# mathcom/G2Vec

Measured on NVIDIA H100. Metric: cbow_context_windows_per_sec, higher is better.
Workload: dtype f32

## Files before the change

### g2vec_b200/_capi.py

```python
import ctypes
import os

from . import build as _build

_lib = None

_vp, _i32, _i64, _u32, _u64, _f32 = (ctypes.c_void_p, ctypes.c_int32, ctypes.c_int64, ctypes.c_uint32,
                                     ctypes.c_uint64, ctypes.c_float)

SIGNATURES = {
    "g2v_abi_version": (ctypes.c_int, []),
    "g2v_last_error": (ctypes.c_char_p, []),
    "g2v_device_info": (ctypes.c_int, [_vp, _vp, _vp, _vp]),
    "g2v_launch_count": (_i64, []),
    "g2v_walk_workspace_bytes": (ctypes.c_size_t, []),
    "g2v_walk_launch": (ctypes.c_int, [_vp, _vp, _vp, _i32, _i64, _i32, _u64, _u32, _i64, _i64, _i64,
                                       _vp, _vp, _vp, _vp]),
    "g2v_walk_packed_bytes": (ctypes.c_int, [_i32, _i64, _vp, _vp]),
    "g2v_walk_prepare": (ctypes.c_int, [_vp, _vp, _vp, _i32, _i64, _vp, _vp, _vp, _vp, _vp]),
    "g2v_walk_launch_packed": (ctypes.c_int, [_vp, _vp, _i32, _i32, _i64, _i32, _u64, _u32, _i64, _i64, _i64,
                                              _vp, _vp, _vp, _vp, _vp]),
    "g2v_walk_host": (ctypes.c_int, [_vp, _vp, _vp, _i32, _i64, _i32, _u64, _u32, _i64, _i64, _i64, _vp, _vp]),
    "g2v_cbow_fwdbwd": (ctypes.c_int, [_vp, _vp, _vp, _vp, _i64, _i64, _f32, _vp, _vp, _vp, _vp, _vp, _vp,
                                       _i32, _i32, _i32, _vp]),
# ... 13 lines not shown
    "g2v_cbow_batch_expand": (ctypes.c_int, [_vp, _vp, _vp, _vp, _i64, _vp, _vp, _i32, _i32, _i32, _vp]),
    "g2v_cbow_epoch_order": (ctypes.c_int, [_vp, _i64, _u64, _i32, _i64, _i64, _vp, _vp]),
    "g2v_cbow_batch_plan_workspace_bytes": (ctypes.c_size_t, [_i64, _i64, _i64, _i32]),
    "g2v_cbow_batch_plan": (ctypes.c_int, [_vp, _vp, _vp, _i64, _i64, _i64, _i32, _vp, _vp, _vp, _vp, _vp, _vp]),
    "g2v_cbow_update": (ctypes.c_int, [_vp, _vp, _vp, _vp, _vp, _vp, _vp, _vp, _i32, _i32, _i32, _f32, _f32,
                                       _f32, _f32, _i32, _vp, _vp]),
    "g2v_cbow_update_nvl": (ctypes.c_int, [_vp, _vp, _vp, _vp, _vp, _vp, _i64, _i32, _i32, _i32, _f32, _f32, _f32,
                                           _f32, _i32, _vp, _vp]),
    "g2v_cbow_adam_tick": (ctypes.c_int, [_vp, _f32, _f32, _f32, _vp]),
    "g2v_cbow_eval": (ctypes.c_int, [_vp, _vp, _vp, _vp, _i64, _i64, _vp, _vp, _vp, _i32, _i32, _i32, _vp]),
    "g2v_cbow_loop_init": (ctypes.c_int, [_vp, _i64, _i32, _vp]),
    "g2v_cbow_loop_attach": (ctypes.c_int, [_vp]),
    "g2v_cbow_loop_begin": (ctypes.c_int, [_vp, _vp, _vp, _vp, _i64, _vp]),
    "g2v_cbow_loop_tail": (ctypes.c_int, [_vp, _vp, _vp, _vp, _vp, _i64, _f32, _vp, _vp, _vp, _vp, _vp, _i32, _i32, _i32,
                                          _vp]),
    "g2v_cbow_loop_decide": (ctypes.c_int, [_vp, _vp, _vp, _vp]),
    "g2v_cbow_loop_counters_nvl": (ctypes.c_int, [_vp, _vp, _vp, _vp, _i32, _vp]),
    "g2v_cbow_slab_plan": (ctypes.c_int, [_i32, _i32, _vp]),
    "g2v_cbow_slab_workspace_bytes": (ctypes.c_size_t, [_i64, _i32, _i32]),
    "g2v_cbow_slab_setup": (ctypes.c_int, [_vp, _vp, _vp, _i64, _i64, _i32, _i32, _vp, _vp]),
    "g2v_cbow_fwdbwd_slabs": (ctypes.c_int, [_vp, _vp, _vp, _i64, _i64, _f32, _vp, _vp, _vp, _vp, _vp, _vp,
                                             _i32, _i32, _i32, _i32, _vp, _vp]),
    "g2v_cbow_eval_slabs": (ctypes.c_int, [_vp, _vp, _vp, _i64, _i64, _vp, _vp, _vp, _i32, _i32, _i32, _i32, _vp, _vp]),
    "g2v_cbow_step_host": (ctypes.c_int, [_vp, _vp, _vp, _i64, _i64, _vp, _vp, _vp, _vp, _vp, _vp, _i32, _i32,
                                          _i32, _i32, _f32, _f32, _f32, _f32, _i32, _vp, _vp]),
    "g2v_cbow_r1_prepare": (ctypes.c_int, [_vp, _vp, _vp, _i32, _i32, _vp]),
    "g2v_cbow_r1_windows": (ctypes.c_int, [_vp, _vp, _vp, _vp, _i64, _i64, _f32, _vp, _vp, _vp, _vp, _i32, _i32, _vp]),
    "g2v_cbow_r1_windows_csc": (ctypes.c_int, [_vp, _vp, _vp, _vp, _i64, _f32, _vp, _vp, _vp, _vp, _vp, _vp, _vp,
                                              _i32, _i32, _vp]),
    "g2v_cbow_r1_scratch_bytes": (ctypes.c_size_t, [_i32]),
    "g2v_cbow_r1_update": (ctypes.c_int, [_vp, _vp, _vp, _vp, _vp, _vp, _vp, _vp, _vp, _i32, _i32, _i32, _f32, _f32,
                                         _f32, _f32, _i32, _vp, _vp]),
    "g2v_pcc_zscore": (ctypes.c_int, [_vp, _i32, _i32, _vp, _vp]),
    "g2v_pcc_edge_weights": (ctypes.c_int, [_vp, _i32, _i32, _vp, _vp, _i64, _vp, _vp]),
    "g2v_paths_canonicalise": (ctypes.c_int, [_vp, _i64, _i32, _vp, _vp, _vp]),
    "g2v_paths_mark": (ctypes.c_int, [_vp, _vp, _vp, _vp, _i64, _i32, _vp, _vp]),
    "g2v_paths_set_workspace_bytes": (ctypes.c_size_t, [_i64]),
    "g2v_paths_set_select": (ctypes.c_int, [_vp, _vp, _vp, _vp, _i64, _i32, _vp, _vp, _vp, _vp]),
    "g2v_paths_set_emit": (ctypes.c_int, [_vp, _vp, _vp, _vp, _i64, _i32, _i32, _vp, _i64, _i64, _vp, _vp, _vp, _vp,
                                          _vp, _vp]),
    "g2v_test_l2_rows": (ctypes.c_int, [_vp, _vp, _vp, _i64, _i32, _i32, _vp, _vp]),
    "g2v_test_draws": (ctypes.c_int, [_u64, _u64, _i32, _vp, _vp]),
    "g2v_test_curand_draws": (ctypes.c_int, [_u64, _u64, _i32, _vp, _vp]),
}

OPT_ADAM_TF1, OPT_SGD = 0, 1
REDUCE_SUM, REDUCE_MEAN = 0, 1
# ... 39 lines not shown
```

### g2vec_b200/cbow.py

```python
import math
import time

import numpy as np
import torch

from . import _capi


def split_indices(n, seed):
    perm = np.arange(n, dtype=np.int64)
    np.random.RandomState(seed).shuffle(perm)
    pivot = int(n * 0.8)
    return perm[:pivot], perm[pivot:]


def truncated_normal(shape, stddev, rng):
    x = rng.standard_normal(size=shape)
    bad = np.abs(x) > 2.0
    while bad.any():
        x[bad] = rng.standard_normal(size=int(bad.sum()))
        bad = np.abs(x) > 2.0
    return (x * stddev).astype(np.float32)


# ... 114 lines not shown
        if n == 0:
            return
        ptr = win.data_ptr()
        for k in [k for k in self._batches if k[0] == ptr]:
            del self._batches[k]
        key = (ptr, n, B)
        for k in [k for k in self._plan_bufs if k[0] == ptr and k != key]:
            del self._plan_bufs[k]
        buf = self._plan_bufs.get(key)
        if buf is None:
            buf = _PlanBuffers(self, win, B)
            self._plan_bufs[key] = buf
        rows, segptr, pos, brp = buf.build(win)
        data = (win, rows, segptr, pos)
        for k in range(brp.shape[0] - 1):
            self._batches[(ptr, k * B, min(B, n - k * B))] = (data, int(brp[k]), int(brp[k + 1] - brp[k]))
        if self._dO is None or self._dO.shape[0] < B:
            self._dO = torch.empty(B, dtype=torch.float32, device=self.device)
        self._pending = None

    def batch_touched(self, win, win_begin, n):
        return self._batches[(self._ptr(win), int(win_begin), int(n))][2]

    def prepare_slabs(self, win, win_begin=0, n_win=None):
        if self.algo != "rows" or self.det:
            return False
        import ctypes
        if not hasattr(self, "_n_slabs"):
            s = ctypes.c_int32(1)
            _capi.check(self.lib.g2v_cbow_slab_plan(self.V, self.D, ctypes.byref(s)), "g2v_cbow_slab_plan")
            self._n_slabs, self._slabs = int(s.value), {}
        n = ((win.shape[0] if win is not None else self.rowptr.shape[0] - 1) - win_begin) if n_win is None else n_win
        if self._n_slabs <= 1 or n <= 0:
            return False
        ws = torch.empty(int(self.lib.g2v_cbow_slab_workspace_bytes(int(n), self.D, self._n_slabs)), dtype=torch.uint8,
                         device=self.device)
        _capi.check(self.lib.g2v_cbow_slab_setup(self.rowptr.data_ptr(), self.gene.data_ptr(), self._ptr(win),
                                                 int(win_begin), int(n), self.V, self._n_slabs, ws.data_ptr(),
                                                 self._stream()), "g2v_cbow_slab_setup")
        self._slabs[(self._ptr(win), int(win_begin), int(n))] = ws
        return True

    def _slab_ws(self, win, win_begin, n):
        slabs = getattr(self, "_slabs", None)
        return slabs.get((self._ptr(win), int(win_begin), int(n))) if slabs else None

    def grad_tensors(self):
        if self.nvl:
            return []
        return [self.g_flat] if self.algo == "rows" else [self.c]

    def exchange(self):
        if self.nvl:
            return "nvl-multicast (multimem.ld_reduce / multimem.st)" if self.nvl["g_mc"] else "nvl-p2p (peer loads / stores)"
        return "nccl all_reduce"

    def _stream(self):
        return torch.cuda.current_stream(self.device).cuda_stream

    @staticmethod
    def _ptr(t):
        return 0 if t is None else t.data_ptr()

    def _csc_for(self, win, win_begin, n):
        csc = getattr(self, "_csc", None)
        if csc is not None and win is not None and csc[0] == win.data_ptr() and win_begin == 0 and n == csc[1]:
            return csc
        return None
# ... 12 lines not shown
                rc = self.lib.g2v_cbow_r1_windows_csc(self.rowptr.data_ptr(), self.gene.data_ptr(),
                                                      self.label.data_ptr(), win.data_ptr(), int(n),
                                                      1.0 / float(n_total), self.s.data_ptr(), csc[2].data_ptr(),
                                                      csc[3].data_ptr(), csc[4].data_ptr(), self.c.data_ptr(),
                                                      self.acc.data_ptr(), self.acc.data_ptr() + 8, self.V,
                                                      self.reduce, self._stream())
                _capi.check(rc, "g2v_cbow_r1_windows_csc")
                return
            rc = self.lib.g2v_cbow_r1_windows(self.rowptr.data_ptr(), self.gene.data_ptr(), self.label.data_ptr(),
                                              self._ptr(win), int(win_begin), int(n), 1.0 / float(n_total),
                                              self.s.data_ptr(), self.c.data_ptr(), self.acc.data_ptr(),
                                              self.acc.data_ptr() + 8, self.V, self.reduce, self._stream())
            _capi.check(rc, "g2v_cbow_r1_windows")
            return
        ws = self._slab_ws(win, win_begin, n)
        if ws is not None:
            rc = self.lib.g2v_cbow_fwdbwd_slabs(self.gene.data_ptr(), self.label.data_ptr(), self._ptr(win),
                                                int(win_begin), int(n), 1.0 / float(n_total), self.W_ih.data_ptr(),
                                                self.W_ho.data_ptr(), self.g_ih.data_ptr(), self.g_ho.data_ptr(),
                                                self.acc.data_ptr(), self.acc.data_ptr() + 8, self.V, self.D,
                                                self.reduce, self._n_slabs, ws.data_ptr(), self._stream())
            _capi.check(rc, "g2v_cbow_fwdbwd_slabs")
            return
        if csc is not None:
            rc = self.lib.g2v_cbow_fwdbwd_csc(self.rowptr.data_ptr(), self.gene.data_ptr(), self.label.data_ptr(),
                                              win.data_ptr(), int(n), 1.0 / float(n_total), self.W_ih.data_ptr(),
                                              self.W_ho.data_ptr(), csc[2].data_ptr(), csc[3].data_ptr(),
                                              csc[4].data_ptr(), self.g_ih.data_ptr(), self.g_ho.data_ptr(),
                                              self.acc.data_ptr(), self.acc.data_ptr() + 8, self.V, self.D,
                                              self.reduce, self._stream())
            _capi.check(rc, "g2v_cbow_fwdbwd_csc")
            return
        rc = self.lib.g2v_cbow_fwdbwd(self.rowptr.data_ptr(), self.gene.data_ptr(), self.label.data_ptr(),
                                      self._ptr(win), int(win_begin), int(n), 1.0 / float(n_total),
                                      self.W_ih.data_ptr(), self.W_ho.data_ptr(), self.g_ih.data_ptr(),
                                      self.g_ho.data_ptr(), self.acc.data_ptr(), self.acc.data_ptr() + 8,
                                      self.V, self.D, self.reduce, self._stream())
        _capi.check(rc, "g2v_cbow_fwdbwd")

    def _plan(self, win, win_begin, n):
        plan = self._batches.get((self._ptr(win), int(win_begin), int(n)))
        if plan is None:
            raise RuntimeError("%s: windows [%d, %d) of this list were not given to prepare_batches"
                               % ("optimizer='lazy_adam'" if self.lazy else "deterministic=True", win_begin, win_begin + n))
        return plan

# ... 86 lines not shown
            nv["hg"].barrier(channel=1)
            return
        rc = self.lib.g2v_cbow_update(self.W_ih.data_ptr(), self.W_ho.data_ptr(), self._ptr(self.m_ih),
                                      self._ptr(self.v_ih), self._ptr(self.m_ho), self._ptr(self.v_ho),
                                      self.g_ih.data_ptr(), self.g_ho.data_ptr(), self.V, self.D, self.opt,
                                      self.lr, self.beta1, self.beta2, self.eps, self.t, adev, self._stream())
        _capi.check(rc, "g2v_cbow_update")

    def evaluate(self, win, slot, win_begin=0, n_win=None):
        n = (win.shape[0] - win_begin) if n_win is None else n_win
        if self.algo == "rank1":
            rc = self.lib.g2v_cbow_r1_windows(self.rowptr.data_ptr(), self.gene.data_ptr(), self.label.data_ptr(),
                                              self._ptr(win), int(win_begin), int(n), 0.0, self.s.data_ptr(), 0, 0,
                                              self.acc.data_ptr() + 8 * slot, self.V, self.reduce, self._stream())
            _capi.check(rc, "g2v_cbow_r1_windows")
            return
        ws = self._slab_ws(win, win_begin, n)
        if ws is not None:
            rc = self.lib.g2v_cbow_eval_slabs(self.gene.data_ptr(), self.label.data_ptr(), self._ptr(win),
                                              int(win_begin), int(n), self.W_ih.data_ptr(), self.W_ho.data_ptr(),
                                              self.acc.data_ptr() + 8 * slot, self.V, self.D, self.reduce,
                                              self._n_slabs, ws.data_ptr(), self._stream())
            _capi.check(rc, "g2v_cbow_eval_slabs")
            return
        rc = self.lib.g2v_cbow_eval(self.rowptr.data_ptr(), self.gene.data_ptr(), self.label.data_ptr(),
                                    self._ptr(win), int(win_begin), int(n), self.W_ih.data_ptr(),
                                    self.W_ho.data_ptr(), self.acc.data_ptr() + 8 * slot, self.V, self.D,
                                    self.reduce, self._stream())
        _capi.check(rc, "g2v_cbow_eval")

    def loss_sum(self, acc_host):
        return float(acc_host[:1].view(torch.float64)[0])


def _nvl_setup(group, n_flat, dev):
    import os
    import sys
    if os.environ.get("G2V_CBOW_NVL", "1") == "0":
        return None
    try:
        import torch.distributed as dist
        import torch.distributed._symmetric_memory as symm
        w = symm.empty(n_flat, dtype=torch.float32, device=dev)
        g = symm.empty(n_flat, dtype=torch.float32, device=dev)
        hw, hg = symm.rendezvous(w, group), symm.rendezvous(g, group)
        mc = os.environ.get("G2V_CBOW_NVL_MULTICAST", "1") != "0"
# ... 263 lines not shown
                                            None if self.result is None else self.result.data_ptr(), m.V * m.D,
                                            self._st()), "g2v_cbow_loop_begin")
        if self.n_tr_loc:
            m.fwdbwd(self.tr_d, self.n_tr)
        if m_fb is not None:
            m_fb.record()
        if dist:
            for g in m.grad_tensors():
                dist.all_reduce(g)
        m.update()
        if m_upd is not None:
            m_upd.record()
        if self.n_va_loc:
            m.evaluate(self.va_d, 2)
        if m_val is not None:
            m_val.record()
        if self.carried and m.det:
            _capi.check(lib.g2v_cbow_loop_tail_det(self.ctl.data_ptr(), m.rowptr.data_ptr(), m.gene.data_ptr(),
                                                   m.label.data_ptr(), self.tr_d.data_ptr(), self.n_tr_loc,
                                                   1.0 / float(self.n_tr), m.W_ih.data_ptr(), m.W_ho.data_ptr(),
                                                   m._csc[4].data_ptr(), m.g_ho.data_ptr(), m.acc.data_ptr(), m.V, m.D,
                                                   m.reduce, m.det_workspace(self.n_tr_loc).data_ptr(), 0, self._st()),
                        "g2v_cbow_loop_tail_det")
        elif self.carried:
            csc = m._csc
            _capi.check(lib.g2v_cbow_loop_tail(self.ctl.data_ptr(), m.rowptr.data_ptr(), m.gene.data_ptr(),
                                               m.label.data_ptr(), self.tr_d.data_ptr(), self.n_tr_loc,
                                               1.0 / float(self.n_tr), m.W_ih.data_ptr(), m.W_ho.data_ptr(),
                                               csc[4].data_ptr(), m.g_ho.data_ptr(), m.acc.data_ptr(), m.V, m.D,
                                               m.reduce, self._st()), "g2v_cbow_loop_tail")
        elif show and self.n_tr_loc:
            m.evaluate(self.tr_d, 3)
        acc_ptr = m.acc.data_ptr()
        if self.hist_nvl:
            hn = self.hist_nvl
            _capi.check(lib.g2v_cbow_loop_counters_nvl(self.ctl.data_ptr(), acc_ptr, hn["h"].buffer_ptrs_dev, hn["mc"],
                                                       m.nvl["world"], self._st()), "g2v_cbow_loop_counters_nvl")
            hn["h"].barrier(channel=3)
            acc_ptr = None
        elif dist:
            dist.all_reduce(m.acc[1:4])
        _capi.check(lib.g2v_cbow_loop_decide(self.ctl.data_ptr(), acc_ptr, self.hist_d.data_ptr(), self._st()),
                    "g2v_cbow_loop_decide")

    def fetch(self):
        self.ctl_pin.copy_(self.ctl, non_blocking=True)
# ... 142 lines not shown
```

### g2vec_b200/csrc/g2v_cbow.cu

```cuda
#include "g2v_cbow_common.cuh"

namespace g2v {

constexpr int kRowsEval = 0, kRowsScatter = 1, kRowsCsc = 2;

template <int VEC, int MODE>
__global__ void __launch_bounds__(kCbowWarps * 32)
cbow_rows_kernel(const int32_t *__restrict__ rowptr, const int32_t *__restrict__ gene,
                 const uint8_t *__restrict__ label, const int32_t *__restrict__ win,
                 int64_t win_begin, int64_t n_win, float inv_n, const float *__restrict__ W_ih,
                 const float *__restrict__ W_ho, float *__restrict__ g_ih, float *__restrict__ g_ho,
                 double *__restrict__ loss_sum, unsigned long long *__restrict__ n_correct,
                 int32_t reduce_mean, const int32_t *__restrict__ skip, float *__restrict__ dO_pos,
                 const int32_t *__restrict__ carried) {
    G2V_SKIP_IF_STOPPED(skip);
    G2V_SKIP_IF_STOPPED(carried);
    constexpr bool BACKWARD = MODE != kRowsEval;
    constexpr int D = 128 * VEC;
    constexpr int D4 = D / 4;
    constexpr int UNR = 8 / VEC;
    __shared__ float sh_gho[BACKWARD ? D : 1];
    __shared__ CtaAcc sh_acc;
    const int lane = threadIdx.x & 31, warp = threadIdx.x >> 5;
    if (BACKWARD) for (int i = threadIdx.x; i < D; i += blockDim.x) sh_gho[i] = 0.f;
// ... 814 lines not shown
}

extern "C" int g2v_cbow_fwd_do(const int32_t *rowptr, const int32_t *gene, const uint8_t *label, const int32_t *win,
                               int64_t n_win, float inv_n_total, const float *W_ih, const float *W_ho, float *dO,
                               float *g_ho, double *loss_sum, int64_t *n_correct, int32_t V, int32_t D, int32_t reduce,
                               void *stream) {
    G2V_REQUIRE(V > 0 && D > 0 && n_win >= 0, "g2v_cbow_fwd_do: bad sizes (V=%d D=%d n_win=%lld)", V, D, (long long)n_win);
    G2V_REQUIRE(rowptr && label && W_ih && W_ho && dO && g_ho, "g2v_cbow_fwd_do: null pointer");
    G2V_REQUIRE(reduce == G2V_REDUCE_SUM || reduce == G2V_REDUCE_MEAN, "g2v_cbow_fwd_do: unknown reduce %d", reduce);
    if (n_win == 0) return 0;
    return launch_rows<true>(rowptr, gene, label, win, 0, n_win, inv_n_total, W_ih, W_ho, nullptr, g_ho, loss_sum,
                             n_correct, D, reduce, (cudaStream_t)stream, dO);
}

extern "C" int g2v_cbow_loop_tail(int64_t *ctl, const int32_t *rowptr, const int32_t *gene, const uint8_t *label,
                                  const int32_t *win, int64_t n_win, float inv_n_total, const float *W_ih,
                                  const float *W_ho, float *dO, float *g_ho, int64_t *acc, int32_t V, int32_t D,
                                  int32_t reduce, void *stream) {
    G2V_REQUIRE(ctl && acc, "g2v_cbow_loop_tail: null loop state");
    cudaStream_t st = (cudaStream_t)stream;
    int rc = g2v_cbow_fwd_do(rowptr, gene, label, win, n_win, inv_n_total, W_ih, W_ho, dO, g_ho,
                             reinterpret_cast<double *>(acc + 4), acc + 5, V, D, reduce, st);
    if (rc) return rc;
    loop_carry_kernel<<<1, 1, 0, st>>>(reinterpret_cast<long long *>(ctl), reinterpret_cast<long long *>(acc));
    G2V_CUDA_OK(cudaGetLastError());
    count_launch();
    return 0;
}

extern "C" size_t g2v_cbow_det_workspace_bytes(int64_t n_win, int32_t D) {
    if (n_win < 0 || D <= 0) return 0;
    const int64_t n_tiles = (n_win + kDetTile - 1) / kDetTile;
    return det_ws_loss_bytes(n_tiles) + (size_t)n_tiles * (size_t)D * sizeof(float);
}

#define G2V_DET_CHECK(name)                                                                                            \
    G2V_REQUIRE(V > 0 && D > 0 && n_win >= 0 && max_ctas >= 0, name ": bad sizes (V=%d D=%d n_win=%lld max_ctas=%d)", \
                V, D, (long long)n_win, max_ctas);                                                                     \
    G2V_REQUIRE(n_win == 0 || (rowptr && gene && label && win && W_ih && W_ho && dO && g_ho && workspace),            \
                name ": null pointer");                                                                                \
    G2V_REQUIRE(reduce == G2V_REDUCE_SUM || reduce == G2V_REDUCE_MEAN, name ": unknown reduce %d", reduce)

extern "C" int g2v_cbow_fwdbwd_csc_det(const int32_t *rowptr, const int32_t *gene, const uint8_t *label,
                                       const int32_t *win, int64_t n_win, float inv_n_total, const float *W_ih,
                                       const float *W_ho, const int32_t *cscptr, const int32_t *csc_pos, float *dO,
                                       float *g_ih, float *g_ho, double *loss_sum, int64_t *n_correct, int32_t V,
// ... 14 lines not shown
}

extern "C" int g2v_cbow_fwd_do_det(const int32_t *rowptr, const int32_t *gene, const uint8_t *label,
                                   const int32_t *win, int64_t n_win, float inv_n_total, const float *W_ih,
                                   const float *W_ho, float *dO, float *g_ho, double *loss_sum, int64_t *n_correct,
                                   int32_t V, int32_t D, int32_t reduce, void *workspace, int32_t max_ctas,
                                   void *stream) {
    G2V_DET_CHECK("g2v_cbow_fwd_do_det");
    if (n_win == 0) return 0;
    return launch_rows_det(rowptr, gene, label, win, n_win, inv_n_total, W_ih, W_ho, dO, g_ho, loss_sum, n_correct, D,
                           reduce, workspace, max_ctas, (cudaStream_t)stream, nullptr);
}
#undef G2V_DET_CHECK

extern "C" int g2v_cbow_loop_tail_det(int64_t *ctl, const int32_t *rowptr, const int32_t *gene, const uint8_t *label,
                                      const int32_t *win, int64_t n_win, float inv_n_total, const float *W_ih,
                                      const float *W_ho, float *dO, float *g_ho, int64_t *acc, int32_t V, int32_t D,
                                      int32_t reduce, void *workspace, int32_t max_ctas, void *stream) {
    G2V_REQUIRE(ctl && acc, "g2v_cbow_loop_tail_det: null loop state");
    cudaStream_t st = (cudaStream_t)stream;
    int rc = g2v_cbow_fwd_do_det(rowptr, gene, label, win, n_win, inv_n_total, W_ih, W_ho, dO, g_ho,
                                 reinterpret_cast<double *>(acc + 4), acc + 5, V, D, reduce, workspace, max_ctas, st);
    if (rc) return rc;
    loop_carry_kernel<<<1, 1, 0, st>>>(reinterpret_cast<long long *>(ctl), reinterpret_cast<long long *>(acc));
    G2V_CUDA_OK(cudaGetLastError());
    count_launch();
    return 0;
}

extern "C" int g2v_cbow_batch_expand(const int32_t *rows, const int32_t *segptr, const int32_t *pos, const float *dO,
                                     int64_t n_rows, const float *W_ho, float *g_ih, int32_t V, int32_t D,
                                     int32_t max_ctas, void *stream) {
    G2V_REQUIRE(V > 0 && D > 0 && n_rows >= 0 && n_rows <= V && max_ctas >= 0,
                "g2v_cbow_batch_expand: bad sizes (V=%d D=%d n_rows=%lld max_ctas=%d)", V, D, (long long)n_rows, max_ctas);
    G2V_REQUIRE(n_rows == 0 || (rows && segptr && pos && dO && W_ho && g_ih), "g2v_cbow_batch_expand: null pointer");
    if (n_rows == 0) return 0;
    int grid = 0, rc;
    if ((rc = det_grid((const void *)cbow_batch_expand_kernel, 0, n_rows, max_ctas, &grid))) return rc;
    cbow_batch_expand_kernel<<<grid, kCbowWarps * 32, 0, (cudaStream_t)stream>>>(rows, segptr, pos, dO, n_rows, W_ho,
                                                                                  g_ih, D, loop_skip_flag());
    G2V_CUDA_OK(cudaGetLastError());
    count_launch();
    return 0;
}

extern "C" int g2v_cbow_eval(const int32_t *rowptr, const int32_t *gene, const uint8_t *label,
                             const int32_t *win, int64_t win_begin, int64_t n_win, const float *W_ih,
                             const float *W_ho, int64_t *n_correct, int32_t V, int32_t D, int32_t reduce,
                             void *stream) {
    G2V_REQUIRE(V > 0 && D > 0 && n_win >= 0 && win_begin >= 0, "g2v_cbow_eval: bad sizes");
// ... 169 lines not shown
```

### g2vec_b200/csrc/g2v_cbow_common.cuh

```cuda
#pragma once
#include "g2v_common.cuh"

namespace g2v {

constexpr int kCbowWarps = 8;

__device__ __forceinline__ float4 ldg4(const float4 *p) { return __ldg(p); }
__device__ __forceinline__ void red_add4(float *p, float4 v) {
    asm volatile("red.global.add.v4.f32 [%0], {%1, %2, %3, %4};" ::"l"(p), "f"(v.x), "f"(v.y), "f"(v.z),
                 "f"(v.w)
                 : "memory");
}
__device__ __forceinline__ float sigmoid_stable(float x) {
    if (x >= 0.f) { const float z = expf(-x); return 1.f / (1.f + z); }
    const float z = expf(x);
    return z / (1.f + z);
}

__device__ __forceinline__ void adam1(float &w, float &m, float &v, float g, float alpha, float omb1,
                                      float omb2, float eps) {
    m += (g - m) * omb1;
    v += (g * g - v) * omb2;
    w -= (m * alpha) / (sqrtf(v) + eps);
}
// ... 16 lines not shown
    constexpr int D = 128 * VEC;
    if (TRAIN && ACTIVE) {
#pragma unroll
        for (int v = 0; v < VEC; ++v) {
            float *p = sh_gho + (v * 32 + lane) * 4;
            atomicAdd(p + 0, gho[v].x); atomicAdd(p + 1, gho[v].y);
            atomicAdd(p + 2, gho[v].z); atomicAdd(p + 3, gho[v].w);
        }
    }
    if (ACTIVE && lane == 0) {
        if (TRAIN) atomicAdd(&sh_acc.loss, (double)loss_acc);
        atomicAdd(&sh_acc.correct, (unsigned long long)correct_acc);
    }
    __syncthreads();
    if (TRAIN && ACTIVE) for (int i = threadIdx.x; i < D; i += blockDim.x) atomicAdd(g_ho + i, sh_gho[i]);
    if (ACTIVE && threadIdx.x == 0) {
        if (TRAIN && loss_sum) atomicAdd(loss_sum, sh_acc.loss);
        if (n_correct) atomicAdd(n_correct, sh_acc.correct);
    }
}

int rows_grid(const void *kernel, size_t smem, int64_t n_items, int *grid_out);

}
```

### include/g2vec_b200.h

```cpp
#ifndef G2VEC_B200_H
#define G2VEC_B200_H

#include <stddef.h>
#include <stdint.h>

#ifdef __cplusplus
extern "C" {
#endif

#define G2V_ABI_VERSION 2

#define G2V_OPT_ADAM_TF1 0
#define G2V_OPT_SGD 1

#define G2V_REDUCE_SUM 0
#define G2V_REDUCE_MEAN 1

int g2v_abi_version(void);
const char *g2v_last_error(void);

int g2v_device_info(int32_t *sm_count, int32_t *cc_major, int32_t *cc_minor, int64_t *l2_bytes);
int64_t g2v_launch_count(void);

size_t g2v_walk_workspace_bytes(void);
// ... 78 lines not shown

int g2v_cbow_loop_init(int64_t *ctl, int64_t max_steps, int32_t early_stop, void *stream);
int g2v_cbow_loop_attach(const int64_t *ctl);
int g2v_cbow_loop_begin(const int64_t *ctl, int64_t *acc, const float *W_ih, float *snapshot, int64_t n, void *stream);
int g2v_cbow_loop_tail(int64_t *ctl, const int32_t *rowptr, const int32_t *gene, const uint8_t *label,
                       const int32_t *win, int64_t n_win, float inv_n_total, const float *W_ih, const float *W_ho,
                       float *dO, float *g_ho, int64_t *acc, int32_t V, int32_t D, int32_t reduce, void *stream);
int g2v_cbow_loop_decide(int64_t *ctl, const int64_t *acc, int64_t *hist, void *stream);
int g2v_cbow_loop_counters_nvl(const int64_t *ctl, const int64_t *acc, int64_t *const *hist_ptrs_dev,
                               int64_t *hist_multicast, int32_t world, void *stream);

int g2v_cbow_slab_plan(int32_t V, int32_t D, int32_t *n_slabs);
size_t g2v_cbow_slab_workspace_bytes(int64_t n_win, int32_t D, int32_t n_slabs);
int g2v_cbow_slab_setup(const int32_t *rowptr, const int32_t *gene, const int32_t *win, int64_t win_begin,
                        int64_t n_win, int32_t V, int32_t n_slabs, void *workspace, void *stream);
int g2v_cbow_fwdbwd_slabs(const int32_t *gene, const uint8_t *label, const int32_t *win, int64_t win_begin,
                          int64_t n_win, float inv_n_total, const float *W_ih, const float *W_ho, float *g_ih,
                          float *g_ho, double *loss_sum, int64_t *n_correct, int32_t V, int32_t D, int32_t reduce,
                          int32_t n_slabs, void *workspace, void *stream);
int g2v_cbow_eval_slabs(const int32_t *gene, const uint8_t *label, const int32_t *win, int64_t win_begin,
                        int64_t n_win, const float *W_ih, const float *W_ho, int64_t *n_correct, int32_t V,
                        int32_t D, int32_t reduce, int32_t n_slabs, void *workspace, void *stream);

int g2v_cbow_step_host(const int32_t *rowptr, const int32_t *gene, const uint8_t *label,
                       int64_t n_win, int64_t nnz, float *W_ih, float *W_ho, float *m_ih,
                       float *v_ih, float *m_ho, float *v_ho, int32_t V, int32_t D,
                       int32_t optimizer, int32_t reduce, float lr, float beta1, float beta2,
                       float eps, int32_t t, double *loss_sum, int64_t *n_correct);

int g2v_cbow_r1_prepare(const float *W_ih, const float *W_ho, float *s, int32_t V, int32_t D,
                        void *stream);
int g2v_cbow_r1_windows(const int32_t *rowptr, const int32_t *gene, const uint8_t *label,
                        const int32_t *win, int64_t win_begin, int64_t n_win, float inv_n_total,
                        const float *s, float *c, double *loss_sum, int64_t *n_correct, int32_t V,
                        int32_t reduce, void *stream);
int g2v_cbow_r1_windows_csc(const int32_t *rowptr, const int32_t *gene, const uint8_t *label,
                            const int32_t *win, int64_t n_win, float inv_n_total, const float *s,
                            const int32_t *cscptr, const int32_t *csc_pos, float *dO, float *c,
                            double *loss_sum, int64_t *n_correct, int32_t V, int32_t reduce, void *stream);
size_t g2v_cbow_r1_scratch_bytes(int32_t D);
int g2v_cbow_r1_update(float *W_ih, float *W_ho, float *m_ih, float *v_ih, float *m_ho, float *v_ho,
                       float *c, float *g_ho, float *s, int32_t V, int32_t D, int32_t optimizer,
                       float lr, float beta1, float beta2, float eps, int32_t t, const float *alpha_dev,
                       void *stream);

int g2v_pcc_zscore(const float *expr, int32_t S, int32_t V, float *z, void *stream);
// ... 26 lines not shown
```

Measured before the change: 153.3 million.

## Add vocabulary-partitioned CBOW forward that stages W_ih row blocks in shared memory

Adds a partitioned CBOW path for vocabularies that fit in a single slab. The path splits the vocabulary into row ranges that fit in shared memory and precomputes per-window split points. Each CTA loads one partition of W_ih into shared memory and sums the partial hidden-output dot products for every window, pulling work chunks through atomic tickets and then moving on to the least-loaded partition. A finish kernel combines the per-partition partial outputs. This replaces scattered global gathers of embedding rows with shared-memory reads, at the cost of a setup pass, extra workspace, and a host sync during setup.

```diff
diff --git a/g2vec_b200/_capi.py b/g2vec_b200/_capi.py
--- a/g2vec_b200/_capi.py
+++ b/g2vec_b200/_capi.py
@@ -59,7 +59,16 @@
     "g2v_cbow_fwdbwd_slabs": (ctypes.c_int, [_vp, _vp, _vp, _i64, _i64, _f32, _vp, _vp, _vp, _vp, _vp, _vp,
                                              _i32, _i32, _i32, _i32, _vp, _vp]),
     "g2v_cbow_eval_slabs": (ctypes.c_int, [_vp, _vp, _vp, _i64, _i64, _vp, _vp, _vp, _i32, _i32, _i32, _i32, _vp, _vp]),
-    "g2v_cbow_step_host": (ctypes.c_int, [_vp, _vp, _vp, _i64, _i64, _vp, _vp, _vp, _vp, _vp, _vp, _i32, _i32,
+    "g2v_cbow_part_plan": (ctypes.c_int, [_i32, _i32, _i32, _vp]),
+    "g2v_cbow_part_workspace_bytes": (ctypes.c_size_t, [_i64, _i32]),
+    "g2v_cbow_part_setup": (ctypes.c_int, [_vp, _vp, _vp, _i64, _i64, _i32, _i32, _vp, _vp, _vp]),
+    "g2v_cbow_fwdbwd_part": (ctypes.c_int, [_vp, _vp, _vp, _i64, _f32, _vp, _vp, _vp, _vp, _vp, _vp, _vp, _vp, _vp,
+                                            _i32, _i32, _i32, _i32, _vp, _i32, _vp]),
+    "g2v_cbow_eval_part": (ctypes.c_int, [_vp, _vp, _vp, _i64, _i64, _vp, _vp, _vp, _i32, _i32, _i32, _i32, _vp, _i32,
+                                          _vp]),
+    "g2v_cbow_loop_tail_part": (ctypes.c_int, [_vp, _vp, _vp, _vp, _i64, _f32, _vp, _vp, _vp, _vp, _i32, _i32, _i32,
+                                               _i32, _vp, _i32, _vp]),
+    "g2v_cbow_step_host":(ctypes.c_int, [_vp, _vp, _vp, _i64, _i64, _vp, _vp, _vp, _vp, _vp, _vp, _i32, _i32,
                                           _i32, _i32, _f32, _f32, _f32, _f32, _i32, _vp, _vp]),
     "g2v_cbow_r1_prepare": (ctypes.c_int, [_vp, _vp, _vp, _i32, _i32, _vp]),
     "g2v_cbow_r1_windows": (ctypes.c_int, [_vp, _vp, _vp, _vp, _i64, _i64, _f32, _vp, _vp, _vp, _vp, _i32, _i32, _vp]),
diff --git a/g2vec_b200/cbow.py b/g2vec_b200/cbow.py
--- a/g2vec_b200/cbow.py
+++ b/g2vec_b200/cbow.py
@@ -160,6 +160,9 @@
     def batch_touched(self, win, win_begin, n):
         return self._batches[(self._ptr(win), int(win_begin), int(n))][2]
 
+    part_rows = 0
+    part_max_ctas = 0
+
     def prepare_slabs(self, win, win_begin=0, n_win=None):
         if self.algo != "rows" or self.det:
             return False
@@ -169,6 +172,8 @@
             _capi.check(self.lib.g2v_cbow_slab_plan(self.V, self.D, ctypes.byref(s)), "g2v_cbow_slab_plan")
             self._n_slabs, self._slabs = int(s.value), {}
         n = ((win.shape[0] if win is not None else self.rowptr.shape[0] - 1) - win_begin) if n_win is None else n_win
+        if self._n_slabs <= 1 and n > 0:
+            self._prepare_parts(win, win_begin, n)
         if self._n_slabs <= 1 or n <= 0:
             return False
         ws = torch.empty(int(self.lib.g2v_cbow_slab_workspace_bytes(int(n), self.D, self._n_slabs)), dtype=torch.uint8,
@@ -182,6 +187,31 @@
     def _slab_ws(self, win, win_begin, n):
         slabs = getattr(self, "_slabs", None)
         return slabs.get((self._ptr(win), int(win_begin), int(n))) if slabs else None
+
+    def _prepare_parts(self, win, win_begin, n):
+        import ctypes
+        if not hasattr(self, "_n_parts"):
+            p = ctypes.c_int32(0)
+            _capi.check(self.lib.g2v_cbow_part_plan(self.V, self.D, int(self.part_rows), ctypes.byref(p)),
+                        "g2v_cbow_part_plan")
+            self._n_parts, self._parts = int(p.value), {}
+        if self._n_parts < 1:
+            return
+        ws = torch.empty(int(self.lib.g2v_cbow_part_workspace_bytes(int(n), self._n_parts)), dtype=torch.uint8,
+                         device=self.device)
+        ok = ctypes.c_int32(0)
+        _capi.check(self.lib.g2v_cbow_part_setup(self.rowptr.data_ptr(), self.gene.data_ptr(), self._ptr(win),
+                                                 int(win_begin), int(n), self.V, self._n_parts, ws.data_ptr(),
+                                                 ctypes.byref(ok), self._stream()), "g2v_cbow_part_setup")
+        key = (self._ptr(win), int(win_begin), int(n))
+        if ok.value:
+            self._parts[key] = ws
+        else:
+            self._parts.pop(key, None)
+
+    def _part_ws(self, win, win_begin, n):
+        parts = getattr(self, "_parts", None)
+        return parts.get((self._ptr(win), int(win_begin), int(n))) if parts else None
 
     def grad_tensors(self):
         if self.nvl:
@@ -240,6 +270,16 @@
                                                 self.reduce, self._n_slabs, ws.data_ptr(), self._stream())
             _capi.check(rc, "g2v_cbow_fwdbwd_slabs")
             return
+        pws = self._part_ws(win, win_begin, n) if csc is not None else None
+        if pws is not None:
+            rc = self.lib.g2v_cbow_fwdbwd_part(self.gene.data_ptr(), self.label.data_ptr(), win.data_ptr(), int(n),
+                                               1.0 / float(n_total), self.W_ih.data_ptr(), self.W_ho.data_ptr(),
+                                               csc[2].data_ptr(), csc[3].data_ptr(), csc[4].data_ptr(),
+                                               self.g_ih.data_ptr(), self.g_ho.data_ptr(), self.acc.data_ptr(),
+                                               self.acc.data_ptr() + 8, self.V, self.D, self.reduce, self._n_parts,
+                                               pws.data_ptr(), int(self.part_max_ctas), self._stream())
+            _capi.check(rc, "g2v_cbow_fwdbwd_part")
+            return
         if csc is not None:
             rc = self.lib.g2v_cbow_fwdbwd_csc(self.rowptr.data_ptr(), self.gene.data_ptr(), self.label.data_ptr(),
                                               win.data_ptr(), int(n), 1.0 / float(n_total), self.W_ih.data_ptr(),
@@ -372,6 +412,14 @@
                                               self.acc.data_ptr() + 8 * slot, self.V, self.D, self.reduce,
                                               self._n_slabs, ws.data_ptr(), self._stream())
             _capi.check(rc, "g2v_cbow_eval_slabs")
+            return
+        pws = self._part_ws(win, win_begin, n)
+        if pws is not None:
+            rc = self.lib.g2v_cbow_eval_part(self.gene.data_ptr(), self.label.data_ptr(), self._ptr(win),
+                                             int(win_begin), int(n), self.W_ih.data_ptr(), self.W_ho.data_ptr(),
+                                             self.acc.data_ptr() + 8 * slot, self.V, self.D, self.reduce,
+                                             self._n_parts, pws.data_ptr(), int(self.part_max_ctas), self._stream())
+            _capi.check(rc, "g2v_cbow_eval_part")
             return
         rc = self.lib.g2v_cbow_eval(self.rowptr.data_ptr(), self.gene.data_ptr(), self.label.data_ptr(),
                                     self._ptr(win), int(win_begin), int(n), self.W_ih.data_ptr(),
@@ -681,6 +729,13 @@
                                                    m._csc[4].data_ptr(), m.g_ho.data_ptr(), m.acc.data_ptr(), m.V, m.D,
                                                    m.reduce, m.det_workspace(self.n_tr_loc).data_ptr(), 0, self._st()),
                         "g2v_cbow_loop_tail_det")
+        elif self.carried and m._part_ws(self.tr_d, 0, self.n_tr_loc) is not None:
+            _capi.check(lib.g2v_cbow_loop_tail_part(self.ctl.data_ptr(), m.gene.data_ptr(), m.label.data_ptr(),
+                                                    self.tr_d.data_ptr(), self.n_tr_loc, 1.0 / float(self.n_tr),
+                                                    m.W_ih.data_ptr(), m.W_ho.data_ptr(), m._csc[4].data_ptr(),
+                                                    m.acc.data_ptr(), m.V, m.D, m.reduce, m._n_parts,
+                                                    m._part_ws(self.tr_d, 0, self.n_tr_loc).data_ptr(),
+                                                    int(m.part_max_ctas), self._st()), "g2v_cbow_loop_tail_part")
         elif self.carried:
             csc = m._csc
             _capi.check(lib.g2v_cbow_loop_tail(self.ctl.data_ptr(), m.rowptr.data_ptr(), m.gene.data_ptr(),
diff --git a/g2vec_b200/csrc/g2v_cbow.cu b/g2vec_b200/csrc/g2v_cbow.cu
--- a/g2vec_b200/csrc/g2v_cbow.cu
+++ b/g2vec_b200/csrc/g2v_cbow.cu
@@ -860,6 +860,10 @@
     int rc = g2v_cbow_fwd_do(rowptr, gene, label, win, n_win, inv_n_total, W_ih, W_ho, dO, g_ho,
                              reinterpret_cast<double *>(acc + 4), acc + 5, V, D, reduce, st);
     if (rc) return rc;
+    return launch_loop_carry(ctl, acc, st);
+}
+
+int g2v::launch_loop_carry(int64_t *ctl, int64_t *acc, cudaStream_t st) {
     loop_carry_kernel<<<1, 1, 0, st>>>(reinterpret_cast<long long *>(ctl), reinterpret_cast<long long *>(acc));
     G2V_CUDA_OK(cudaGetLastError());
     count_launch();
@@ -920,10 +924,7 @@
     int rc = g2v_cbow_fwd_do_det(rowptr, gene, label, win, n_win, inv_n_total, W_ih, W_ho, dO, g_ho,
                                  reinterpret_cast<double *>(acc + 4), acc + 5, V, D, reduce, workspace, max_ctas, st);
     if (rc) return rc;
-    loop_carry_kernel<<<1, 1, 0, st>>>(reinterpret_cast<long long *>(ctl), reinterpret_cast<long long *>(acc));
-    G2V_CUDA_OK(cudaGetLastError());
-    count_launch();
-    return 0;
+    return launch_loop_carry(ctl, acc, st);
 }
 
 extern "C" int g2v_cbow_batch_expand(const int32_t *rows, const int32_t *segptr, const int32_t *pos, const float *dO,
diff --git a/g2vec_b200/csrc/g2v_cbow_common.cuh b/g2vec_b200/csrc/g2v_cbow_common.cuh
--- a/g2vec_b200/csrc/g2v_cbow_common.cuh
+++ b/g2vec_b200/csrc/g2v_cbow_common.cuh
@@ -62,4 +62,6 @@
 
 int rows_grid(const void *kernel, size_t smem, int64_t n_items, int *grid_out);
 
+int launch_loop_carry(int64_t *ctl, int64_t *acc, cudaStream_t st);
+
 }
diff --git a/g2vec_b200/csrc/g2v_cbow_part.cu b/g2vec_b200/csrc/g2v_cbow_part.cu
--- /dev/null
+++ b/g2vec_b200/csrc/g2v_cbow_part.cu
@@ -0,0 +1,427 @@
+#include <stdlib.h>
+
+#include "g2v_cbow_common.cuh"
+
+namespace g2v {
+
+constexpr int kPartWarps = 32;
+constexpr int kPartChunk = 32;
+constexpr int kPartStaticSmem = 256;
+constexpr int kPartMaxP = 32;
+
+__global__ void __launch_bounds__(256)
+part_setup_kernel(const int32_t *__restrict__ rowptr, const int32_t *__restrict__ gene,
+                  const int32_t *__restrict__ win, int64_t win_begin, int64_t n_win, int32_t V, int32_t rows, int32_t P,
+                  int32_t *__restrict__ spT, int32_t *__restrict__ bad) {
+    for (int64_t i = (int64_t)blockIdx.x * blockDim.x + threadIdx.x; i < n_win; i += (int64_t)gridDim.x * blockDim.x) {
+        const int64_t n = win ? (int64_t)__ldg(win + win_begin + i) : win_begin + i;
+        const int32_t b = __ldg(rowptr + n), e = __ldg(rowptr + n + 1);
+        int s = 0;
+        int32_t prev = 0;
+        spT[i] = b;
+        for (int32_t j = b; j < e; ++j) {
+            const int32_t g = __ldg(gene + j);
+            if (g < prev || g >= V) *bad = 1;
+            prev = g;
+            while (s + 1 <= P - 1 && g >= (s + 1) * rows) spT[(int64_t)(++s) * n_win + i] = j;
+        }
+        while (s < P) spT[(int64_t)(++s) * n_win + i] = e;
+    }
+}
+
+template <int VEC>
+__global__ void __launch_bounds__(kPartWarps * 32, 1)
+cbow_part_fwd_kernel(const int32_t *__restrict__ gene, const int32_t *__restrict__ spT, int64_t n_win, int32_t P,
+                     int32_t rows, int32_t V, const float *__restrict__ W_ih, const float *__restrict__ W_ho,
+                     float *__restrict__ obuf, int32_t *__restrict__ tickets, int32_t reduce_mean,
+                     const int32_t *__restrict__ skip, const int32_t *__restrict__ carried) {
+    G2V_SKIP_IF_STOPPED(skip);
+    G2V_SKIP_IF_STOPPED(carried);
+    constexpr int D = 128 * VEC;
+    constexpr int D4 = D / 4;
+    constexpr int GR = VEC == 4 ? 1 : 8 / VEC;
+    extern __shared__ float4 sh_rows[];
+    __shared__ int32_t sh_next;
+    const int lane = threadIdx.x & 31;
+    const int64_t n_chunks = (n_win + kPartChunk - 1) / kPartChunk;
+    float4 who[VEC];
+#pragma unroll
+    for (int v = 0; v < VEC; ++v) who[v] = ldg4(reinterpret_cast<const float4 *>(W_ho) + v * 32 + lane);
+
+    int32_t p = (int32_t)(blockIdx.x % (unsigned)P);
+    for (;;) {
+        const int32_t lo = p * rows;
+        const int32_t n_rows = min(rows, V - lo);
+        const float4 *__restrict__ src = reinterpret_cast<const float4 *>(W_ih) + (size_t)lo * D4;
+        for (int k = threadIdx.x; k < n_rows * D4; k += blockDim.x) sh_rows[k] = ldg4(src + k);
+        __syncthreads();
+        const int32_t *__restrict__ sp_b = spT + (int64_t)p * n_win;
+        const int32_t *__restrict__ sp_e = sp_b + n_win;
+        int64_t c = 0;
+        if (lane == 0) c = atomicAdd(tickets + p, 1);
+        c = __shfl_sync(0xffffffffu, c, 0);
+        while (c < n_chunks) {
+            int64_t c_next = 0;
+            if (lane == 0) c_next = atomicAdd(tickets + p, 1);
+            const int64_t i0 = c * kPartChunk, i = i0 + lane;
+            int32_t b = 0, e = 0;
+            float scl = 1.f;
+            if (i < n_win) {
+                b = __ldg(sp_b + i);
+                e = __ldg(sp_e + i);
+                if (reduce_mean) {
+                    const int32_t len = __ldg(spT + (int64_t)P * n_win + i) - __ldg(spT + i);
+                    scl = len > 0 ? 1.f / (float)len : 1.f;
+                }
+            }
+            int32_t g[GR];
+#pragma unroll
+            for (int u = 0; u < GR; ++u) g[u] = (b + u < e) ? __ldg(gene + b + u) - lo : 0;
+            float my_o = 0.f, part_prev = 0.f;
+            int k_prev = -1;
+            const int kn = (int)min((int64_t)kPartChunk, n_win - i0);
+            for (int k = 0; k < kn; ++k) {
+                const int32_t cnt = __shfl_sync(0xffffffffu, e - b, k);
+                float4 h[VEC];
+#pragma unroll
+                for (int v = 0; v < VEC; ++v) h[v] = make_float4(0.f, 0.f, 0.f, 0.f);
+#pragma unroll
+                for (int u = 0; u < (GR < 4 ? GR : 4); ++u) {
+                    const int32_t gk = __shfl_sync(0xffffffffu, g[u], k);
+                    const float4 *row = sh_rows + (size_t)gk * D4 + lane;
+#pragma unroll
+                    for (int v = 0; v < VEC; ++v) {
+                        const float4 r = (u < cnt) ? row[v * 32] : make_float4(0.f, 0.f, 0.f, 0.f);
+                        h[v].x += r.x; h[v].y += r.y; h[v].z += r.z; h[v].w += r.w;
+                    }
+                }
+                {
+                    const float o = warp_sum(part_prev);
+                    if (lane == k_prev) my_o = o;
+                }
+                if (GR > 4 && cnt > 4) {
+#pragma unroll
+                    for (int u = 4; u < GR; ++u) {
+                        const int32_t gk = __shfl_sync(0xffffffffu, g[u], k);
+                        const float4 *row = sh_rows + (size_t)gk * D4 + lane;
+#pragma unroll
+                        for (int v = 0; v < VEC; ++v) {
+                            const float4 r = (u < cnt) ? row[v * 32] : make_float4(0.f, 0.f, 0.f, 0.f);
+                            h[v].x += r.x; h[v].y += r.y; h[v].z += r.z; h[v].w += r.w;
+                        }
+                    }
+                }
+                if (cnt > GR) {
+                    const int32_t bk = __shfl_sync(0xffffffffu, b, k), ek = bk + cnt;
+                    for (int32_t base = bk + GR; base < ek; base += 32) {
+                        const int m = min(32, ek - base);
+                        const int32_t gl = lane < m ? __ldg(gene + base + lane) - lo : 0;
+                        for (int kk = 0; kk < m; ++kk) {
+                            const int32_t gk = __shfl_sync(0xffffffffu, gl, kk);
+                            const float4 *row = sh_rows + (size_t)gk * D4 + lane;
+#pragma unroll
+                            for (int v = 0; v < VEC; ++v) {
+                                const float4 r = row[v * 32];
+                                h[v].x += r.x; h[v].y += r.y; h[v].z += r.z; h[v].w += r.w;
+                            }
+                        }
+                    }
+                }
+                const float scale = reduce_mean ? __shfl_sync(0xffffffffu, scl, k) : 1.f;
+                float part = 0.f;
+#pragma unroll
+                for (int v = 0; v < VEC; ++v) {
+                    if (reduce_mean) { h[v].x *= scale; h[v].y *= scale; h[v].z *= scale; h[v].w *= scale; }
+                    part += h[v].x * who[v].x + h[v].y * who[v].y + h[v].z * who[v].z + h[v].w * who[v].w;
+                }
+                part_prev = part;
+                k_prev = k;
+            }
+            const float o = warp_sum(part_prev);
+            if (lane == k_prev) my_o = o;
+            if (i < n_win) obuf[(int64_t)p * n_win + i] = my_o;
+            c = __shfl_sync(0xffffffffu, c_next, 0);
+        }
+        __syncthreads();
+        if (threadIdx.x == 0) {
+            int32_t best = -1;
+            int64_t least = n_chunks;
+            for (int32_t q = 0; q < P; ++q) {
+                const int64_t t = *reinterpret_cast<const volatile int32_t *>(tickets + q);
+                if (t < least) { least = t; best = q; }
+            }
+            sh_next = best;
+        }
+        __syncthreads();
+        p = sh_next;
+        if (p < 0) break;
+    }
+}
+
+template <bool TRAIN>
+__global__ void __launch_bounds__(256)
+cbow_part_finish_kernel(const uint8_t *__restrict__ label, const int32_t *__restrict__ win, int64_t win_begin,
+                        int64_t n_win, const int32_t *__restrict__ spT, int32_t P, const float *__restrict__ obuf,
+                        float inv_n, float *__restrict__ dO_pos, double *__restrict__ loss_sum,
+                        unsigned long long *__restrict__ n_correct, int32_t *__restrict__ tickets, int32_t reduce_mean,
+                        const int32_t *__restrict__ skip, const int32_t *__restrict__ carried) {
+    G2V_SKIP_IF_STOPPED(skip);
+    G2V_SKIP_IF_STOPPED(carried);
+    __shared__ CtaAcc sh_acc;
+    if (threadIdx.x == 0) { sh_acc.loss = 0.0; sh_acc.correct = 0ull; }
+    if (blockIdx.x == 0)
+        for (int q = threadIdx.x; q < P; q += blockDim.x) tickets[q] = 0;
+    __syncthreads();
+    float loss_acc = 0.f;
+    unsigned correct_acc = 0;
+    for (int64_t i = (int64_t)blockIdx.x * blockDim.x + threadIdx.x; i < n_win; i += (int64_t)gridDim.x * blockDim.x) {
+        float o = __ldg(obuf + i);
+        for (int32_t p = 1; p < P; ++p) o += __ldg(obuf + (int64_t)p * n_win + i);
+        const int64_t n = win ? (int64_t)__ldg(win + win_begin + i) : win_begin + i;
+        const float y = (float)__ldg(label + n);
+        correct_acc += ((o > 0.f) == (y != 0.f)) ? 1u : 0u;
+        if (TRAIN) {
+            loss_acc += fmaxf(o, 0.f) - o * y + log1pf(expf(-fabsf(o)));
+            const int32_t len = __ldg(spT + (int64_t)P * n_win + i) - __ldg(spT + i);
+            const float scale = (reduce_mean && len > 0) ? 1.f / (float)len : 1.f;
+            const float dO = (sigmoid_stable(o) - y) * inv_n;
+            dO_pos[i] = dO * scale;
+        }
+    }
+    const float l = warp_sum(loss_acc);
+    const unsigned long long c = warp_sum_u64(correct_acc);
+    if ((threadIdx.x & 31) == 0) {
+        if (TRAIN) atomicAdd(&sh_acc.loss, (double)l);
+        atomicAdd(&sh_acc.correct, c);
+    }
+    __syncthreads();
+    if (threadIdx.x == 0) {
+        if (TRAIN && loss_sum) atomicAdd(loss_sum, sh_acc.loss);
+        if (n_correct) atomicAdd(n_correct, sh_acc.correct);
+    }
+}
+
+template <int VEC>
+__global__ void __launch_bounds__(kCbowWarps * 32)
+cbow_part_expand_kernel(const int32_t *__restrict__ cscptr, const int32_t *__restrict__ csc_pos,
+                        const float *__restrict__ dO_pos, const float *__restrict__ W_ih,
+                        const float *__restrict__ W_ho, float *__restrict__ g_ih, float *__restrict__ g_ho, int32_t V,
+                        const int32_t *__restrict__ skip) {
+    G2V_SKIP_IF_STOPPED(skip);
+    constexpr int D = 128 * VEC;
+    constexpr int D4 = D / 4;
+    __shared__ float sh_gho[D];
+    __shared__ CtaAcc sh_acc;
+    const int lane = threadIdx.x & 31;
+    for (int i = threadIdx.x; i < D; i += blockDim.x) sh_gho[i] = 0.f;
+    if (threadIdx.x == 0) { sh_acc.loss = 0.0; sh_acc.correct = 0ull; }
+    __syncthreads();
+    float4 who[VEC], gho[VEC];
+#pragma unroll
+    for (int v = 0; v < VEC; ++v) {
+        who[v] = ldg4(reinterpret_cast<const float4 *>(W_ho) + v * 32 + lane);
+        gho[v] = make_float4(0.f, 0.f, 0.f, 0.f);
+    }
+    const int64_t warp = (int64_t)blockIdx.x * kCbowWarps + (threadIdx.x >> 5);
+    const int64_t nwarps = (int64_t)gridDim.x * kCbowWarps;
+    for (int64_t g = warp; g < V; g += nwarps) {
+        const int32_t b = __ldg(cscptr + g), e = __ldg(cscptr + g + 1);
+        if (b == e) continue;
+        const float c = csc_segment_sum(csc_pos, dO_pos, b, e, lane);
+        float4 *r4 = reinterpret_cast<float4 *>(g_ih) + (size_t)g * D4 + lane;
+        const float4 *w4 = reinterpret_cast<const float4 *>(W_ih) + (size_t)g * D4 + lane;
+#pragma unroll
+        for (int v = 0; v < VEC; ++v) {
+            const float4 w = who[v], x = ldg4(w4 + v * 32);
+            float4 a = r4[v * 32];
+            a.x += c * w.x; a.y += c * w.y; a.z += c * w.z; a.w += c * w.w;
+            r4[v * 32] = a;
+            gho[v].x += c * x.x; gho[v].y += c * x.y; gho[v].z += c * x.z; gho[v].w += c * x.w;
+        }
+    }
+    cta_epilogue<VEC, true, true>(sh_gho, sh_acc, gho, 0.f, 0u, lane, g_ho, nullptr, nullptr);
+}
+
+struct PartLayout {
+    int32_t *spT;
+    float *obuf;
+    int32_t *tickets;
+};
+
+static size_t align256(size_t x) { return (x + 255) & ~(size_t)255; }
+
+static PartLayout carve(void *ws, int64_t n_win, int32_t P) {
+    char *p = reinterpret_cast<char *>(ws);
+    PartLayout l;
+    l.spT = reinterpret_cast<int32_t *>(p); p += align256(sizeof(int32_t) * (size_t)n_win * (size_t)(P + 1));
+    l.obuf = reinterpret_cast<float *>(p); p += align256(sizeof(float) * (size_t)n_win * (size_t)P);
+    l.tickets = reinterpret_cast<int32_t *>(p);
+    return l;
+}
+
+static int32_t part_rows(int32_t V, int32_t P) { return (V + P - 1) / P; }
+
+static int capped_grid(int64_t want, int32_t max_ctas) {
+    if (max_ctas > 0 && want > max_ctas) want = max_ctas;
+    return (int)(want > 0 ? want : 1);
+}
+
+template <bool TRAIN>
+static int launch_part_forward(const int32_t *gene, const uint8_t *label, const int32_t *win, int64_t win_begin,
+                               int64_t n_win, float inv_n, const float *W_ih, const float *W_ho, float *dO,
+                               double *loss_sum, unsigned long long *nc, int32_t V, int32_t D, int32_t reduce,
+                               int32_t P, void *workspace, int32_t max_ctas, cudaStream_t st, const int32_t *carried) {
+    DeviceProps dp;
+    if (device_props(&dp)) return 1;
+    if (dp.cc_major != 9) { set_error("needs an sm_90 device (found sm_%d%d); no CPU fallback", dp.cc_major, dp.cc_minor); return 2; }
+    PartLayout l = carve(workspace, n_win, P);
+    const int32_t rows = part_rows(V, P);
+    const size_t smem = (size_t)rows * D * sizeof(float);
+    G2V_REQUIRE(smem + kPartStaticSmem <= (size_t)dp.max_smem_optin,
+                "cbow partition of %d rows x %d does not fit the shared memory (%d B)", rows, D, dp.max_smem_optin);
+    const int64_t work = (n_win + kPartChunk - 1) / kPartChunk * P;
+    const int grid = capped_grid(work < dp.sm_count ? work : dp.sm_count, max_ctas);
+#define G2V_PART_FWD(VEC)                                                                                              \
+    {                                                                                                                  \
+        auto kern = cbow_part_fwd_kernel<VEC>;                                                                         \
+        G2V_CUDA_OK(cudaFuncSetAttribute(kern, cudaFuncAttributeMaxDynamicSharedMemorySize, (int)smem));               \
+        kern<<<grid, kPartWarps * 32, smem, st>>>(gene, l.spT, n_win, P, rows, V, W_ih, W_ho, l.obuf, l.tickets,      \
+                                                   reduce, loop_skip_flag(), carried);                                 \
+    }
+    if (D == 128) G2V_PART_FWD(1)
+    else if (D == 256) G2V_PART_FWD(2)
+    else G2V_PART_FWD(4)
+#undef G2V_PART_FWD
+    G2V_CUDA_OK(cudaGetLastError());
+    const int64_t fblocks = (n_win + 255) / 256;
+    const int fgrid = capped_grid(fblocks < dp.sm_count * 4 ? fblocks : dp.sm_count * 4, max_ctas);
+    cbow_part_finish_kernel<TRAIN><<<fgrid, 256, 0, st>>>(label, win, win_begin, n_win, l.spT, P, l.obuf, inv_n, dO,
+                                                          loss_sum, nc, l.tickets, reduce, loop_skip_flag(), carried);
+    G2V_CUDA_OK(cudaGetLastError());
+    count_launch(2);
+    return 0;
+}
+
+#define G2V_PART_CHECK(name)                                                                                           \
+    G2V_REQUIRE(V > 0 && n_win >= 0 && n_parts >= 1 && n_parts <= V && max_ctas >= 0,                                 \
+                name ": bad sizes (V=%d n_win=%lld n_parts=%d max_ctas=%d)", V, (long long)n_win, n_parts, max_ctas);  \
+    G2V_REQUIRE(D == 128 || D == 256 || D == 512, name ": sizeHiddenlayer must be 128, 256 or 512 (got %d)", D);      \
+    G2V_REQUIRE(reduce == G2V_REDUCE_SUM || reduce == G2V_REDUCE_MEAN, name ": unknown reduce %d", reduce)
+
+}
+
+using namespace g2v;
+
+extern "C" int g2v_cbow_part_plan(int32_t V, int32_t D, int32_t rows_per_part, int32_t *n_parts) {
+    G2V_REQUIRE(V > 0 && D > 0 && rows_per_part >= 0 && n_parts, "g2v_cbow_part_plan: bad arguments");
+    *n_parts = 0;
+    DeviceProps dp;
+    if (device_props(&dp)) return 1;
+    if (D != 128 && D != 256 && D != 512) return 0;
+    const char *f = getenv("G2V_CBOW_SLABS");
+    if (f && atoi(f) >= 1) return 0;
+    if ((double)V * D * 4.0 > 0.9 * (double)dp.l2_bytes) return 0;
+    const int32_t fit = (dp.max_smem_optin - kPartStaticSmem) / (4 * D);
+    G2V_REQUIRE(fit >= 1 && rows_per_part <= fit, "g2v_cbow_part_plan: %d rows of %d floats do not fit the shared "
+                "memory (at most %d)", rows_per_part, D, fit);
+    if (rows_per_part > 0) { *n_parts = (V + rows_per_part - 1) / rows_per_part; return 0; }
+    const int32_t P = (V + fit - 1) / fit;
+    if (P >= 2 && P <= kPartMaxP) *n_parts = P;
+    return 0;
+}
+
+extern "C" size_t g2v_cbow_part_workspace_bytes(int64_t n_win, int32_t n_parts) {
+    if (n_win <= 0 || n_parts <= 0) return 0;
+    return align256(sizeof(int32_t) * (size_t)n_win * (size_t)(n_parts + 1)) +
+           align256(sizeof(float) * (size_t)n_win * (size_t)n_parts) + align256(sizeof(int32_t) * (size_t)(n_parts + 1));
+}
+
+extern "C" int g2v_cbow_part_setup(const int32_t *rowptr, const int32_t *gene, const int32_t *win, int64_t win_begin,
+                                   int64_t n_win, int32_t V, int32_t n_parts, void *workspace, int32_t *sorted,
+                                   void *stream) {
+    G2V_REQUIRE(V > 0 && n_parts >= 1 && n_parts <= V && n_win >= 0 && win_begin >= 0 && sorted,
+                "g2v_cbow_part_setup: bad sizes");
+    *sorted = 1;
+    if (n_win == 0) return 0;
+    G2V_REQUIRE(rowptr && gene && workspace, "g2v_cbow_part_setup: null pointer");
+    DeviceProps dp;
+    if (device_props(&dp)) return 1;
+    cudaStream_t st = (cudaStream_t)stream;
+    PartLayout l = carve(workspace, n_win, n_parts);
+    int32_t *bad = l.tickets + n_parts;
+    G2V_CUDA_OK(cudaMemsetAsync(l.tickets, 0, sizeof(int32_t) * (size_t)(n_parts + 1), st));
+    int64_t blocks = (n_win + 255) / 256;
+    if (blocks > (int64_t)dp.sm_count * 8) blocks = (int64_t)dp.sm_count * 8;
+    part_setup_kernel<<<(unsigned)blocks, 256, 0, st>>>(rowptr, gene, win, win_begin, n_win, V, part_rows(V, n_parts),
+                                                        n_parts, l.spT, bad);
+    G2V_CUDA_OK(cudaGetLastError());
+    count_launch();
+    int32_t h = 0;
+    G2V_CUDA_OK(cudaMemcpyAsync(&h, bad, sizeof(int32_t), cudaMemcpyDeviceToHost, st));
+    G2V_CUDA_OK(cudaStreamSynchronize(st));
+    *sorted = h == 0;
+    return 0;
+}
+
+extern "C" int g2v_cbow_fwdbwd_part(const int32_t *gene, const uint8_t *label, const int32_t *win, int64_t n_win,
+                                    float inv_n_total, const float *W_ih, const float *W_ho, const int32_t *cscptr,
+                                    const int32_t *csc_pos, float *dO, float *g_ih, float *g_ho, double *loss_sum,
+                                    int64_t *n_correct, int32_t V, int32_t D, int32_t reduce, int32_t n_parts,
+                                    void *workspace, int32_t max_ctas, void *stream) {
+    G2V_PART_CHECK("g2v_cbow_fwdbwd_part");
+    G2V_REQUIRE(n_win == 0 || (gene && label && W_ih && W_ho && cscptr && csc_pos && dO && g_ih && g_ho && workspace),
+                "g2v_cbow_fwdbwd_part: null pointer");
+    if (n_win == 0) return 0;
+    cudaStream_t st = (cudaStream_t)stream;
+    int rc = launch_part_forward<true>(gene, label, win, 0, n_win, inv_n_total, W_ih, W_ho, dO, loss_sum,
+                                       reinterpret_cast<unsigned long long *>(n_correct), V, D, reduce, n_parts,
+                                       workspace, max_ctas, st, loop_carry_flag());
+    if (rc) return rc;
+    int grid = 0;
+#define G2V_PART_EXPAND(VEC)                                                                                           \
+    {                                                                                                                  \
+        if ((rc = rows_grid((const void *)cbow_part_expand_kernel<VEC>, 0, V, &grid))) return rc;                      \
+        grid = capped_grid(grid, max_ctas);                                                                            \
+        cbow_part_expand_kernel<VEC><<<grid, kCbowWarps * 32, 0, st>>>(cscptr, csc_pos, dO, W_ih, W_ho, g_ih, g_ho, V, \
+                                                                       loop_skip_flag());                              \
+    }
+    if (D == 128) G2V_PART_EXPAND(1)
+    else if (D == 256) G2V_PART_EXPAND(2)
+    else G2V_PART_EXPAND(4)
+#undef G2V_PART_EXPAND
+    G2V_CUDA_OK(cudaGetLastError());
+    count_launch();
+    return 0;
+}
+
+extern "C" int g2v_cbow_eval_part(const int32_t *gene, const uint8_t *label, const int32_t *win, int64_t win_begin,
+                                  int64_t n_win, const float *W_ih, const float *W_ho, int64_t *n_correct, int32_t V,
+                                  int32_t D, int32_t reduce, int32_t n_parts, void *workspace, int32_t max_ctas,
+                                  void *stream) {
+    G2V_PART_CHECK("g2v_cbow_eval_part");
+    G2V_REQUIRE(win_begin >= 0, "g2v_cbow_eval_part: bad win_begin");
+    G2V_REQUIRE(n_win == 0 || (gene && label && W_ih && W_ho && n_correct && workspace), "g2v_cbow_eval_part: null pointer");
+    if (n_win == 0) return 0;
+    return launch_part_forward<false>(gene, label, win, win_begin, n_win, 0.f, W_ih, W_ho, nullptr, nullptr,
+                                      reinterpret_cast<unsigned long long *>(n_correct), V, D, reduce, n_parts,
+                                      workspace, max_ctas, (cudaStream_t)stream, nullptr);
+}
+
+extern "C" int g2v_cbow_loop_tail_part(int64_t *ctl, const int32_t *gene, const uint8_t *label, const int32_t *win,
+                                       int64_t n_win, float inv_n_total, const float *W_ih, const float *W_ho,
+                                       float *dO, int64_t *acc, int32_t V, int32_t D, int32_t reduce, int32_t n_parts,
+                                       void *workspace, int32_t max_ctas, void *stream) {
+    G2V_REQUIRE(ctl && acc, "g2v_cbow_loop_tail_part: null loop state");
+    G2V_PART_CHECK("g2v_cbow_loop_tail_part");
+    G2V_REQUIRE(n_win == 0 || (gene && label && W_ih && W_ho && dO && workspace), "g2v_cbow_loop_tail_part: null pointer");
+    cudaStream_t st = (cudaStream_t)stream;
+    if (n_win > 0) {
+        int rc = launch_part_forward<true>(gene, label, win, 0, n_win, inv_n_total, W_ih, W_ho, dO,
+                                           reinterpret_cast<double *>(acc + 4),
+                                           reinterpret_cast<unsigned long long *>(acc + 5), V, D, reduce, n_parts,
+                                           workspace, max_ctas, st, nullptr);
+        if (rc) return rc;
+    }
+    return launch_loop_carry(ctl, acc, st);
+}
+#undef G2V_PART_CHECK
diff --git a/include/g2vec_b200.h b/include/g2vec_b200.h
--- a/include/g2vec_b200.h
+++ b/include/g2vec_b200.h
@@ -124,6 +124,23 @@
                         int64_t n_win, const float *W_ih, const float *W_ho, int64_t *n_correct, int32_t V,
                         int32_t D, int32_t reduce, int32_t n_slabs, void *workspace, void *stream);
 
+int g2v_cbow_part_plan(int32_t V, int32_t D, int32_t rows_per_part, int32_t *n_parts);
+size_t g2v_cbow_part_workspace_bytes(int64_t n_win, int32_t n_parts);
+int g2v_cbow_part_setup(const int32_t *rowptr, const int32_t *gene, const int32_t *win, int64_t win_begin,
+                        int64_t n_win, int32_t V, int32_t n_parts, void *workspace, int32_t *sorted, void *stream);
+int g2v_cbow_fwdbwd_part(const int32_t *gene, const uint8_t *label, const int32_t *win, int64_t n_win,
+                         float inv_n_total, const float *W_ih, const float *W_ho, const int32_t *cscptr,
+                         const int32_t *csc_pos, float *dO, float *g_ih, float *g_ho, double *loss_sum,
+                         int64_t *n_correct, int32_t V, int32_t D, int32_t reduce, int32_t n_parts, void *workspace,
+                         int32_t max_ctas, void *stream);
+int g2v_cbow_eval_part(const int32_t *gene, const uint8_t *label, const int32_t *win, int64_t win_begin,
+                       int64_t n_win, const float *W_ih, const float *W_ho, int64_t *n_correct, int32_t V, int32_t D,
+                       int32_t reduce, int32_t n_parts, void *workspace, int32_t max_ctas, void *stream);
+int g2v_cbow_loop_tail_part(int64_t *ctl, const int32_t *gene, const uint8_t *label, const int32_t *win,
+                            int64_t n_win, float inv_n_total, const float *W_ih, const float *W_ho, float *dO,
+                            int64_t *acc, int32_t V, int32_t D, int32_t reduce, int32_t n_parts, void *workspace,
+                            int32_t max_ctas, void *stream);
+
 int g2v_cbow_step_host(const int32_t *rowptr, const int32_t *gene, const uint8_t *label,
                        int64_t n_win, int64_t nnz, float *W_ih, float *W_ho, float *m_ih,
                        float *v_ih, float *m_ho, float *v_ho, int32_t V, int32_t D,
```

Result: faster. 192.8 million, median of 6 (+25.8%).
